# yanyan-li/Structure-SLAM-PointLine

Measured on AMD Instinct MI355X. Metric: front-end frames/sec (ORB+LSD extract+match) 640x480 @1000kp/200ln, higher is better.
Workload: dtype u8; 1 GPU; BASELINE configs[2]: 640x480 ORB(1000kp,8 levels)+LSD/LBD(<=200 lines) extract + Hamming match vs previous frame, inputs resident in HBM; batch_per_gpu=12288, global_batch=12288, unique_frames=64, streams=point branch and line branch on two HIP streams, parallelism=single GPU

## Files before the change

### include/sslam_testing.h

```cpp
#ifndef SSLAM_TESTING_H
#define SSLAM_TESTING_H
#include "sslam_frontend.h"
#ifdef __cplusplus
extern "C" {
#endif

int sslam_testing_use_rccl_standin(int on);

int sslam_selftest_exact_div(sslam_ctx* ctx, int n, long long pairs, long long* mismatches_out);
int sslam_debug_nfa_tables(int n, double* out);
int sslam_selftest_tail_test(sslam_ctx* ctx, long long samples, long long* disagree_out, long long* ambiguous_out);
int sslam_selftest_region_div(sslam_ctx* ctx, long long samples, long long mismatches_out[2]);

int sslam_selftest_sincos(sslam_ctx* ctx, long long* mismatches_out);
int sslam_selftest_lsd_bin(sslam_ctx* ctx, int max_s, long long* mismatches_out);
int sslam_selftest_lbd_round(sslam_ctx* ctx, long long mismatches_out[2]);

int sslam_selftest_valu_rate(sslam_ctx* ctx, int kind, double* ginst_per_s_out);
int sslam_selftest_fetch_probe(sslam_ctx* ctx, size_t bytes, int mode, long long* bytes_requested_out);
int sslam_lines_debug_cluster(sslam_lines* ln, int frame, long long* out8);


#ifdef __cplusplus
}
#endif
#endif
```

### structure-slam-pointline_amd/csrc/lbd.h

```cpp
#pragma once

template <class KeyPtr>
__device__ __forceinline__ void keyline_sort(KeyPtr keys, int P2, int tid) {
    for (int k = 2; k <= P2; k <<= 1)
        for (int j = k >> 1; j > 0; j >>= 1) {
            for (int i = tid; i < P2; i += 256) {
                int ixj = i ^ j;
                if (ixj > i) {
                    unsigned long long a = keys[i], c = keys[ixj];
                    bool up = (i & k) == 0;
                    if ((a > c) == up) { keys[i] = c; keys[ixj] = a; }
                }
            }
            __syncthreads();
        }
}

constexpr int KL_LDS = 1024;
__global__ __launch_bounds__(256) void k_keylines(uint8_t* __restrict__ ws, LsdPlan P, int maxLines,
                                                  sslam_keyline* __restrict__ klOut, double* __restrict__ fnOut,
                                                  int* __restrict__ counts, int cap) {
    __shared__ unsigned long long keysL[KL_LDS];
    const int b = blockIdx.x, tid = threadIdx.x;
    uint8_t* base = ws + (size_t)b * P.frameBytes;
// ... 33 lines not shown
        const float W = (float)P.w, H = (float)P.h;
        if (e0 < 0) e0 = 0; if (e0 >= W) e0 = W - 1.0f;
        if (e2 < 0) e2 = 0; if (e2 >= W) e2 = W - 1.0f;
        if (e1 < 0) e1 = 0; if (e1 >= H) e1 = H - 1.0f;
        if (e3 < 0) e3 = 0; if (e3 >= H) e3 = H - 1.0f;
        sslam_keyline k;
        k.startPointX = e0; k.startPointY = e1; k.endPointX = e2; k.endPointY = e3;
        k.sPointInOctaveX = e0; k.sPointInOctaveY = e1; k.ePointInOctaveX = e2; k.ePointInOctaveY = e3;
        const double ddx = (double)__fsub_rn(e0, e2), ddy = (double)__fsub_rn(e1, e3);
        k.lineLength = (float)sqrt(ddx * ddx + ddy * ddy);
        const int ax = cv_roundf(e0), ay = cv_roundf(e1), bx = cv_roundf(e2), by = cv_roundf(e3);
        k.numOfPixels = max(abs(bx - ax), abs(by - ay)) + 1;
        k.angle = (float)atan2((double)__fsub_rn(e3, e1), (double)__fsub_rn(e2, e0));
        k.class_id = i; k.octave = 0;
        k.size = __fmul_rn(__fsub_rn(e2, e0), __fsub_rn(e3, e1));
        k.response = __fdiv_rn(k.lineLength, (float)max(P.w, P.h));
        k.pt_x = __fdiv_rn(__fadd_rn(e2, e0), 2.f); k.pt_y = __fdiv_rn(__fadd_rn(e3, e1), 2.f);
        klw[i] = k;
        const unsigned long long key = ((unsigned long long)(~__float_as_uint(k.response)) << 32) | (unsigned)i;
        if (inLds) keysL[i] = key; else keysG[i] = key;
    }
    __syncthreads();
    int nOut = n;
    const bool doSort = n > maxLines;
    if (doSort) {
        int P2 = 1; while (P2 < n) P2 <<= 1;
        if (inLds) {
            for (int i = n + tid; i < P2; i += 256) keysL[i] = ~0ull;
            __syncthreads();
            keyline_sort(keysL, P2, tid);
        } else {
            for (int i = n + tid; i < P2; i += 256) keysG[i] = ~0ull;
            __syncthreads();
            keyline_sort(keysG, P2, tid);
        }
        nOut = maxLines;
    }
    nOut = min(nOut, cap);
    for (int i = tid; i < nOut; i += 256) {
        const int src = doSort ? (int)(unsigned)(inLds ? keysL[i] : keysG[i]) : i;
        sslam_keyline k = klw[src];
        if (doSort) k.class_id = i;
        klOut[(size_t)b * cap + i] = k;
        ((float2*)(base + P.offLbdDir))[i] = make_float2((float)cos((double)k.angle), (float)sin((double)k.angle));
        const double sx = k.startPointX, sy = k.startPointY, ex = k.endPointX, ey = k.endPointY;
        const double l0 = __dsub_rn(sy, ey), l1 = __dsub_rn(ex, sx), l2 = __dsub_rn(__dmul_rn(sx, ey), __dmul_rn(sy, ex));
        const double nrm = sqrt(__dadd_rn(__dmul_rn(l0, l0), __dmul_rn(l1, l1)));
        double* f = fnOut + ((size_t)b * cap + i) * 3;
        f[0] = l0 / nrm; f[1] = l1 / nrm; f[2] = l2 / nrm;
    }
    if (tid == 0) { counts[b] = nOut; misc->nKl = nOut; }
}

__global__ __launch_bounds__(256) void k_blur_sobel(const uint8_t* __restrict__ src, size_t spitch, size_t sframe, int w, int h,
                                                    unsigned* __restrict__ dxyo, size_t dframeBytes,
                                                    const int* __restrict__ tapsArr) {
    constexpr int R = 3;
    const int ngroups = (w + 3) >> 2;
    const int t = blockIdx.x * 256 + threadIdx.x;
    const int strip = t / ngroups, x4 = (t - strip * ngroups) * 4, y0 = strip * STRIP;
    if (y0 >= h) return;
    const int b = blockIdx.y;
    const uint8_t* s = src + (size_t)b * sframe;
    unsigned taps[5];
#pragma unroll
    for (int k = 0; k < 5; ++k) taps[k] = (unsigned)tapsArr[k];
    const unsigned T0 = taps[0] | (taps[1] << 8) | (taps[2] << 16) | (taps[3] << 24), T1 = taps[4];
    const bool fast = x4 >= 4 && x4 + 8 <= w && ((spitch | (size_t)(uintptr_t)s) & 3) == 0;
    const bool vec = ((w & 3) == 0) && ((dframeBytes & 15) == 0);
    unsigned hb[5][6];
    int bl[3][6];
    constexpr int NR = STRIP + 2 * R;
    const bool uni = row12_uniform(s, spitch, w);
    const int x4u = uni ? x4 : 0;
    Row12 ring[ROW_AHEAD_SOBEL];
#pragma unroll
    for (int k = 0; k < ROW_AHEAD_SOBEL; ++k) ring[k] = row12_issue(s, spitch, reflect_row(y0 - R + k, h, R), x4u, w);
#pragma unroll
    for (int r = 0; r < NR; ++r) {
        if (r >= 2 * R && y0 + r - 2 * R >= h) break;
        Row12 cur = ring[r % ROW_AHEAD_SOBEL];
        if (r + ROW_AHEAD_SOBEL < NR) ring[r % ROW_AHEAD_SOBEL] = row12_issue(s, spitch, reflect_row(y0 - R + r + ROW_AHEAD_SOBEL, h, R), x4u, w);
        row12_fix(cur, x4u, w);
        if (!uni) load_row12(s, spitch, reflect_row(y0 - R + r, h, R), x4, w, fast, cur.d0, cur.d1, cur.d2);
        const unsigned d0 = cur.d0, d1 = cur.d1, d2 = cur.d2;
#pragma unroll
        for (int c = 0; c < 6; ++c) hb[r % 5][c] = hdot(d0, d1, d2, c + 1, T0, T1);
        if (r >= 4) {
            const int q = r - 4;
#pragma unroll
            for (int c = 0; c < 6; ++c) {
                unsigned acc = 0;
#pragma unroll
                for (int k = 0; k < 5; ++k) acc = __umul24(hb[(q + k) % 5][c], taps[k]) + acc;
                bl[q % 3][c] = (int)min((acc + 32768u) >> 16, 255u);
            }
            if (q >= 2) {
                const int y = y0 + q - 2;
                const int* A = bl[(q - 2) % 3];
                const int* M = bl[(q - 1) % 3];
                const int* C = bl[q % 3];
                short gx[4], gy[4];
#pragma unroll
                for (int j = 0; j < 4; ++j) {
                    gx[j] = (short)((A[j + 2] - A[j]) + 2 * (M[j + 2] - M[j]) + (C[j + 2] - C[j]));
                    gy[j] = (short)((C[j] - A[j]) + 2 * (C[j + 1] - A[j + 1]) + (C[j + 2] - A[j + 2]));
                }
                unsigned* op = (unsigned*)((uint8_t*)dxyo + (size_t)b * dframeBytes) + (size_t)y * w + x4;
                unsigned pk[4];
#pragma unroll
                for (int j = 0; j < 4; ++j) pk[j] = ((unsigned)(unsigned short)gx[j]) | ((unsigned)(unsigned short)gy[j] << 16);
                if (x4 + 3 < w && vec) *(uint4*)op = make_uint4(pk[0], pk[1], pk[2], pk[3]);
                else {
#pragma unroll
                    for (int j = 0; j < 4; ++j) if (x4 + j < w) op[j] = pk[j];
                }
            }
        }
    }
}

__constant__ float kGaussL[21];
__constant__ float kGaussL2[21];
__constant__ float kGaussG[63];
__constant__ signed char kComb[64];

typedef float f32x2 __attribute__((ext_vector_type(2)));
__device__ __forceinline__ int cvt_rpi(float x) { int r; asm("v_cvt_rpi_i32_f32 %0, %1" : "=v"(r) : "v"(x)); return r; }
__device__ __forceinline__ f32x2 pk_mul_lo(f32x2 a, f32x2 b) { f32x2 r; asm("v_pk_mul_f32 %0, %1, %2 op_sel:[0,0] op_sel_hi:[1,0]" : "=v"(r) : "v"(a), "v"(b)); return r; }
__device__ __forceinline__ f32x2 pk_mul_hi_swapped(f32x2 a, f32x2 b) { f32x2 r; asm("v_pk_mul_f32 %0, %1, %2 op_sel:[1,1] op_sel_hi:[0,1]" : "=v"(r) : "v"(a), "v"(b)); return r; }
__device__ __forceinline__ f32x2 pk_add_sub(f32x2 a, f32x2 b) { f32x2 r; asm("v_pk_add_f32 %0, %1, %2 neg_hi:[0,1]" : "=v"(r) : "v"(a), "v"(b)); return r; }
__device__ __forceinline__ f32x2 pk_sub(f32x2 a, f32x2 b) { f32x2 r; asm("v_pk_add_f32 %0, %1, %2 neg_lo:[0,1] neg_hi:[0,1]" : "=v"(r) : "v"(a), "v"(b)); return r; }
__device__ __forceinline__ float max0(float x) { float r; asm("v_max_f32 %0, 0, %1" : "=v"(r) : "v"(x)); return r; }
__device__ __forceinline__ int med3_0(int x, int hi) { int r; asm("v_med3_i32 %0, %1, 0, %2" : "=v"(r) : "v"(x), "s"(hi)); return r; }
__device__ __forceinline__ f32x2 pk_mul(f32x2 a, f32x2 b) { f32x2 r; asm("v_pk_mul_f32 %0, %1, %2" : "=v"(r) : "v"(a), "v"(b)); return r; }
__device__ __forceinline__ f32x2 pk_add(f32x2 a, f32x2 b) { f32x2 r; asm("v_pk_add_f32 %0, %1, %2" : "=v"(r) : "v"(a), "v"(b)); return r; }

#ifdef SSLAM_TESTING
__global__ __launch_bounds__(256) void k_selftest_lbd_round(unsigned long long* __restrict__ bad) {
    unsigned long long nb0 = 0, nb1 = 0;
    const unsigned base = (blockIdx.x * 256u + threadIdx.x) << 8;
    for (unsigned i = 0; i < 256u; ++i) {
        const float x = __uint_as_float(base + i);
        if (!(fabsf(x) < 24608.f)) continue;
        const int t = (int)__fadd_rn(x, x);
        const int o = (int)(short)((t + 1) >> 1), n = cvt_rpi(x);
        const int Ws[3] = {0, 639, 16383};
#pragma unroll
        for (int k = 0; k < 3; ++k) nb0 += (min(max(o, 0), Ws[k]) != min(max(n, 0), Ws[k])) ? 1 : 0;
        if (x >= 0.f) nb1 += (n != (int)roundf(x)) ? 1 : 0;
    }
    if (nb0) atomicAdd(bad, nb0);
    if (nb1) atomicAdd(bad + 1, nb1);
}
#endif
constexpr int LBD_TB = 8;
template <bool RPI>
__global__ __launch_bounds__(64) void k_lbd(const uint8_t* __restrict__ ws, LsdPlan P, const sslam_keyline* __restrict__ kls,
                                            const int* __restrict__ counts, uint8_t* __restrict__ descOut, int cap) {
    constexpr int TB = LBD_TB, TN = TB, TP = TB + 1;
    __shared__ unsigned tbuf[64 * TP];
    float (*rows)[64] = (float (*)[64])&tbuf[0];
    static_assert(8 * 64 <= 64 * TP, "rows[][] lies over the walk's block array");
    __shared__ float band[8][NUM_BANDS];
    __shared__ float des[72];
    const int li = blockIdx.x, b = blockIdx.y, lane = threadIdx.x;
    if (li >= counts[b]) return;
    const uint8_t* base = ws + (size_t)b * P.frameBytes;
    const unsigned* dxyImg = (const unsigned*)(base + P.offDxy);
    const sslam_keyline kl = kls[(size_t)b * cap + li];
    const int lengthOfLSP = (short)kl.numOfPixels;
// ... 177 lines not shown
```

### structure-slam-pointline_amd/csrc/lines.hip

```cpp
#include "common.h"
#include <cmath>
#include <cstdlib>
#include <cfloat>
#include <algorithm>

namespace sslam { int launch_nfa_stream(sslam_ctx* ctx, hipStream_t st, uint8_t* ws, const void* plan, size_t planBytes, const double* lgam, uint8_t* clArea, size_t clFrameBytes,
                                        size_t stageOff, int nframes, int waves, long long spinTicks, bool besideCore); }
namespace sslam { int launch_nfa_stage(sslam_ctx* ctx, hipStream_t st, uint8_t* ws, const void* plan, size_t planBytes, const double* lgam, int nframes); }

using namespace sslam;

namespace {

#include "lsd_plan.h"
#include "lsd_front.h"
#include "lsd_regions.h"
#include "lsd_cluster.h"
#include "lsd_nfa.h"
#include "lbd.h"

__global__ void k_zero_misc(uint8_t* ws, LsdPlan P) {
    Misc* m = (Misc*)(ws + (size_t)blockIdx.x * P.frameBytes + P.offMisc);
    if (threadIdx.x == 0) {
        m->maxS = 0; m->nDefined = 0; m->nSeg = 0; m->nCand = 0; m->nKl = 0; m->overflow = 0; m->claim = 0;
#if defined(SSLAM_LSD_DRIFT_VERIFY) || defined(SSLAM_LSD_CYCLES)
        m->cyc[5] = 0; m->cyc[6] = 0; m->cyc[7] = 0;
#endif
    }
}

__global__ __launch_bounds__(256) void k_lines_status(const uint8_t* __restrict__ ws, LsdPlan P, int nframes, int maxLines, int cap, int* __restrict__ status) {
    __shared__ int cnt[2], first[2];
    if (threadIdx.x < 2) { cnt[threadIdx.x] = 0; first[threadIdx.x] = 0x7FFFFFFF; }
    __syncthreads();
    for (int b = threadIdx.x; b < nframes; b += 256) {
        const Misc* m = (const Misc*)(ws + (size_t)b * P.frameBytes + P.offMisc);
        if (min(m->nSeg, maxLines) > cap) { atomicAdd(&cnt[0], 1); atomicMin(&first[0], b); }
        if (m->overflow) { atomicAdd(&cnt[1], 1); atomicMin(&first[1], b); }
    }
    __syncthreads();
    if (threadIdx.x == 0) { status[0] = cnt[0]; status[1] = first[0]; status[2] = cnt[1]; status[3] = first[1]; }
}

}

struct sslam_lines {
    sslam_ctx* ctx;
    int maxLines;
    int planW = 0, planH = 0;
    LsdPlan plan;
    DevBuf dWs, dTabs, dTaps, dLgam, dGtab;
    size_t clFrame = 0; int clSlots = 0;
    DevBuf dCl;
    int wsFrames = 0, lastFrames = 0;
    hipEvent_t coreEvent = nullptr;
    hipEvent_t coreWait = nullptr, coreDone = nullptr;
    int lastN = -1;
    DevBuf dImg, dKl, dDesc, dFn, dCounts;
    HostPinned hOut;
    bool constsUploaded = false;
    int blurVariant = 0;
    int nfaVariant = 1, lbdBitOrder = 1, lsdResize = 0;
    int seedOrder = 0;
    int sMin = 0;
    bool fusedGeometry = false;
    hipStream_t nfaStream = nullptr; hipEvent_t nfaFork = nullptr, nfaJoin = nullptr;
};

static std::vector<int> taps_q8(int n, double sigma) {
    std::vector<double> k(n);
    double sum = 0, s2 = -0.5 / (sigma * sigma);
    for (int i = 0; i < n; ++i) { double x = i - (n - 1) * 0.5; k[i] = std::exp(s2 * x * x); sum += k[i]; }
    std::vector<int> t(n);
    double err = 0; long isum = 0;
    for (int i = 0; i < n / 2; ++i) {
        double adj = k[i] / sum * 256.0 + err;
        int v = (int)lrint(adj);
        err = adj - v; t[i] = t[n - 1 - i] = v; isum += v;
    }
    t[n / 2] = (int)(256 - 2 * isum);
    return t;
}

static std::vector<int> taps_340(int n, double sigma) {
    std::vector<float> k(n); double sum = 0; const double s2 = -0.5 / (sigma * sigma);
    for (int i = 0; i < n; ++i) { const double x = i - (n - 1) * 0.5; k[i] = (float)std::exp(s2 * x * x); sum += k[i]; }
    sum = 1. / sum;
    std::vector<int> t(n);
    for (int i = 0; i < n; ++i) { k[i] = (float)(k[i] * sum); t[i] = (int)lrint((double)k[i] * 256.0); }
    return t;
}

static size_t align_up(size_t v, size_t a) { return (v + a - 1) / a * a; }

static int lines_build_plan(sslam_lines* L, int w, int h) {
    LsdPlan& P = L->plan;
    memset(&P, 0, sizeof(P));
    P.w = w; P.h = h;
    const double SCALE = 0.8;
    P.sw = (int)lrint(w * SCALE); P.sh = (int)lrint(h * SCALE);
    if (P.sw < 8 || P.sh < 8) { set_error("image %dx%d too small for LSD", w, h); return SSLAM_ERR_UNSUPPORTED; }
    P.spitch = (P.sw + 63) & ~63;
    P.npx = P.sw * P.sh;
    if (P.sw > 65535 || P.sh > 65535) { set_error("image %dx%d too large", w, h); return SSLAM_ERR_UNSUPPORTED; }
    P.nXB = (P.sw + 255) / 256;
    P.tileRows = std::min(64, std::max(1, TILE_PX / P.sw));
    P.nTiles = (P.sh + P.tileRows - 1) / P.tileRows;
    if (P.tileRows * P.nXB > MAX_TSEG) { set_error("image %dx%d: too many segments per counting-sort tile", w, h); return SSLAM_ERR_UNSUPPORTED; }
    const double ANG_TH = 22.5, QUANT = 2.0, SIGMA_SCALE = 0.6;
    P.prec = kPI * ANG_TH / 180; P.p = ANG_TH / 180;
    P.rho = QUANT / std::sin(P.prec);
    P.logNT = 5 * (std::log10((double)P.sw) + std::log10((double)P.sh)) / 2 + std::log10(11.0);
    P.minRegSize = (int)(size_t)(-P.logNT / std::log10(P.p));
    const double sigma = SIGMA_SCALE / SCALE;
    const unsigned hk = (unsigned)std::ceil(sigma * std::sqrt(2 * 3.0 * std::log(10.0)));
    if (hk != 3) { set_error("unexpected LSD kernel size"); return SSLAM_ERR_UNSUPPORTED; }
    std::vector<int> t7 = L->blurVariant == 1 ? taps_340(7, sigma) : taps_q8(7, sigma), t5 = L->blurVariant == 1 ? taps_340(5, 1.0) : taps_q8(5, 1.0);
    for (int t : t7) if (t < 0 || t > 255) { set_error("blur taps do not fit a byte"); return SSLAM_ERR_UNSUPPORTED; }
    for (int t : t5) if (t < 0 || t > 255) { set_error("blur taps do not fit a byte"); return SSLAM_ERR_UNSUPPORTED; }
// ... 144 lines not shown
    int nfaStreamWaves;
    long long nfaSpinTicks;
};
static LinesKnobs lines_knobs() {
    LinesKnobs K{-1, true, 0, 10, 640 / CL_SUB, 0, 16, 5000000};
    if (const char* e = getenv("SSLAM_LSD_FLAVOUR")) { K.lone = e[0] == 'l' || e[0] == 'c'; K.cluster = e[0] == 'c'; }
    if (const char* e = getenv("SSLAM_LSD_CLUSTER")) K.cluster = K.cluster && atoi(e) != 0;
    if (const char* e = getenv("SSLAM_LSD_PERSIST")) { const int g = atoi(e) & ~7; if (g >= 8) K.persist = g; }
    if (const char* e = getenv("SSLAM_CL_WGS")) K.clWgs = std::max(1, std::min(CL_MAXWG, atoi(e)));
    if (const char* e = getenv("SSLAM_CL_WINDOW")) K.clWindow = std::max(-1, atoi(e));
    if (getenv("SSLAM_CL_NO_FEEDER") && K.clWindow >= 0) K.clWindow |= 1 << 20;
    if (const char* e = getenv("SSLAM_CL_SMAP")) K.clSmap = atoi(e);
    if (const char* e = getenv("SSLAM_NFA_STREAM")) { const int n = atoi(e); K.nfaStreamWaves = std::max(0, std::min(64, n == 1 ? 16 : n)); }
    if (const char* e = getenv("SSLAM_NFA_STREAM_TICKS")) K.nfaSpinTicks = std::max(0ll, atoll(e));
    return K;
}

static bool lines_guest_form(const sslam_lines* L, int nframes, const LinesKnobs& K, int* grid_out) {
    int grid = 18 * L->ctx->num_cus;
    if (2 * grid > nframes) grid = 16 * L->ctx->num_cus;
    if (K.persist) grid = K.persist;
    if (grid_out) *grid_out = grid;
    return L->coreEvent != nullptr && nframes >= 1024 && 2 * grid <= nframes;
}
extern "C" int sslam_lines_core_guest_form(sslam_lines* L, int nframes) {
    if (!L || nframes <= 0) return 0;
    return lines_guest_form(L, nframes, lines_knobs(), nullptr) ? 1 : 0;
}

enum class CoreForm {
    ClusterStream,
    Cluster,
    Lone,
    Guest,
    PerFrame,
    SixWave,
};

constexpr int CL_MAXFRAMES = 64;

static CoreForm lines_core_form(const sslam_lines* L, const LsdPlan& P, int nframes, const LinesKnobs& K, int* grid) {
    if (K.cluster && nframes <= CL_MAXFRAMES && P.sw <= TorusGlobal::XMASK + 1 && P.sh <= TorusGlobal::YMASK + 1)
        return K.nfaStreamWaves ? CoreForm::ClusterStream : CoreForm::Cluster;
    if (K.lone >= 0 ? K.lone != 0 : nframes < 1024) return CoreForm::Lone;
    if (lines_guest_form(L, nframes, K, grid)) return CoreForm::Guest;
    return nframes <= 16 * L->ctx->num_cus ? CoreForm::PerFrame : CoreForm::SixWave;
}

extern "C" int sslam_lines_destroy(sslam_lines* L) {
    if (!L) return SSLAM_OK;
    (void)hipSetDevice(L->ctx->device);
    (void)hipStreamSynchronize(L->ctx->stream);
    if (L->nfaStream) { (void)hipStreamSynchronize(L->nfaStream); (void)hipStreamDestroy(L->nfaStream); (void)hipEventDestroy(L->nfaFork); (void)hipEventDestroy(L->nfaJoin); }
    DevBuf* bufs[] = {&L->dWs, &L->dCl, &L->dTabs, &L->dTaps, &L->dLgam, &L->dGtab, &L->dImg, &L->dKl, &L->dDesc, &L->dFn, &L->dCounts};
    for (DevBuf* b : bufs) b->release();
    L->hOut.release();
    delete L;
    return SSLAM_OK;
}

struct LinesCall {
    sslam_lines* L; const LsdPlan& P; const uint8_t* images; size_t pitch, imageStride; int nframes; hipStream_t st; uint8_t* ws;
};

struct SideJoin {
    sslam_lines* L; hipStream_t st; bool forked = false, joined = false;
    void join() { if (forked && !joined) { (void)hipEventRecord(L->nfaJoin, L->nfaStream); (void)hipStreamWaitEvent(st, L->nfaJoin, 0); joined = true; } }
    ~SideJoin() { join(); }
};

static int lines_side_stream_ready(sslam_lines* L) {
    if (!L->nfaStream) {
        SSLAM_HIP(hipStreamCreateWithFlags(&L->nfaStream, hipStreamNonBlocking));
        SSLAM_HIP(hipEventCreateWithFlags(&L->nfaFork, hipEventDisableTiming));
        SSLAM_HIP(hipEventCreateWithFlags(&L->nfaJoin, hipEventDisableTiming));
    }
    return SSLAM_OK;
}

static void lines_blur_sobel(const LinesCall& c, hipStream_t s) {
    const LsdPlan& P = c.P;
    sslam::ProfScope _ps(c.L->ctx, "k_blur_sobel", s);
    hipLaunchKernelGGL(k_blur_sobel, dim3((((P.w + 3) / 4) * ((P.h + STRIP - 1) / STRIP) + 255) / 256, c.nframes), dim3(256), 0, s, c.images, c.pitch, c.imageStride, P.w, P.h,
                       (unsigned*)(c.ws + P.offDxy), P.frameBytes, c.L->dTaps.as<int>() + 8);
}

static int lines_prologue(const LinesCall& c) {
    sslam_lines* L = c.L; const LsdPlan& P = c.P; hipStream_t st = c.st;
    const int* taps = L->dTaps.as<int>();
    const int* tabX = L->dTabs.as<int>() + P.tabX; const int* tabY = L->dTabs.as<int>() + P.tabY;
    const int mode = (P.lsdResize ? 1 : 0) | (L->seedOrder ? 2 : 0);
    const bool fused = L->fusedGeometry && GRAD_ROWS == 8 && ((uintptr_t)c.images & 3) == 0 && (c.pitch & 3) == 0 && (c.imageStride & 3) == 0 && c.pitch <= 0x7FFFFFFF;
    if (fused) {
        static decltype(&k_lsd_grad_fused<0>) const kGradFused[4] = {k_lsd_grad_fused<0>, k_lsd_grad_fused<1>, k_lsd_grad_fused<2>, k_lsd_grad_fused<3>};
        sslam::ProfScope _ps(L->ctx, "k_lsd_grad", st);
        const dim3 gg(P.nXB, (P.sh + 31) / 32, c.nframes);
        hipLaunchKernelGGL(kGradFused[mode], gg, dim3(64, 4), 0, st, c.images, c.pitch, c.imageStride, c.ws, P, L->dGtab.as<float4>(), tabX, tabY, taps, c.nframes);
    } else {
        static decltype(&k_lsd_grad<0>) const kGrad[4] = {k_lsd_grad<0>, k_lsd_grad<1>, k_lsd_grad<2>, k_lsd_grad<3>};
        const size_t bpitch = ((size_t)P.w + 63) & ~(size_t)63;
        { sslam::ProfScope _ps(L->ctx, "k_blur7", st); hipLaunchKernelGGL(k_blur7, dim3((((P.w + 3) / 4) * ((P.h + STRIP - 1) / STRIP) + 255) / 256, c.nframes), dim3(256), 0, st, c.images, c.pitch, c.imageStride,
                           c.ws + P.offBlur, bpitch, P.frameBytes, P.w, P.h, taps); }
        { sslam::ProfScope _ps(L->ctx, "k_lsd_grad", st);
          const dim3 gg(P.nXB, (P.sh + 4 * GRAD_ROWS - 1) / (4 * GRAD_ROWS), c.nframes);
          hipLaunchKernelGGL(kGrad[mode], gg, dim3(64, 4), 0, st, c.ws, P, L->dGtab.as<float4>(), bpitch, tabX, tabY); }
    }
    if (L->seedOrder) return lines_host_seed_order(L, c.ws, c.nframes, st);
    const bool runs = P.sw <= (1 << SORT_XY_BITS) && P.sh <= (1 << SORT_XY_BITS);
    const dim3 sg(sort_grid(P.nTiles, c.nframes));
    { sslam::ProfScope _ps(L->ctx, "k_lsd_hist", st); hipLaunchKernelGGL(runs ? k_lsd_hist_sort : k_lsd_hist, sg, dim3(64), 0, st, c.ws, P, c.nframes); }
    { sslam::ProfScope _ps(L->ctx, "k_lsd_scan", st); hipLaunchKernelGGL(k_lsd_scan, dim3(c.nframes), dim3(1024), 0, st, c.ws, P); }
    { sslam::ProfScope _ps(L->ctx, "k_lsd_scatter", st); hipLaunchKernelGGL(runs ? k_lsd_scatter_runs : k_lsd_scatter, sg, dim3(64), 0, st, c.ws, P, c.nframes); }
    return SSLAM_OK;
}

static int lines_core_cluster(const LinesCall& c, const LinesKnobs& K, bool streamNfa, SideJoin& side, size_t* nfaStageOff) {
    sslam_lines* L = c.L; const LsdPlan& P = c.P; const int nframes = c.nframes; hipStream_t st = c.st;
    int rc;
    const bool bigFrame = P.sw > TorusFrame::XMASK + 1 || P.sh > TorusFrame::YMASK + 1;
    const int window = K.clWindow, clShift = K.clSmap;
    int nWG = K.clWgs;
    const int clSpecWords = clShift < 0 ? 0 : (((P.sw + (1 << clShift) - 1) >> clShift) * ((P.sh + (1 << clShift) - 1) >> clShift) + 31) / 32;
    const size_t maxSubs = ((size_t)P.npx + CL_SUB - 1) / CL_SUB;
    const size_t zeroBytes = 512 + ((maxSubs * sizeof(ClSub) + 511) & ~(size_t)511) + 4 * (size_t)((clSpecWords + 127) & ~127) + (bigFrame ? 4 * (size_t)TorusGlobal::WORDS : 0);
    if (nframes > 8) nWG = std::max(2, std::min(nWG, 32 / ((nframes + 7) / 8)));
    const size_t stageOff = zeroBytes + maxSubs * CL_RES * sizeof(ClRec) + 4 * (size_t)CL_ARENA * (size_t)std::max(1, (nWG - 1) * CL_HPW);
    const size_t clFrame = align_up(stageOff + (streamNfa ? sizeof(double) * 12 * (size_t)MAX_SEG : 0), 4096);
    L->clFrame = clFrame; L->clSlots = nframes;
    const size_t clSlots = (size_t)nframes;
    if (L->dCl.cap < clFrame * clSlots) { SSLAM_HIP(hipStreamSynchronize(st)); if ((rc = L->dCl.ensure(clFrame * clSlots))) return rc; }
    for (int f = 0; f < nframes; ++f) SSLAM_HIP(hipMemsetAsync(L->dCl.as<uint8_t>() + (size_t)f * clFrame, 0, zeroBytes, st));
    const size_t clLds = sizeof(unsigned) * std::max((size_t)QCAP + 4 + (bigFrame ? 0 : TorusFrame::WORDS) + CL_SCAN + CL_RING_WORDS, (size_t)CL_HPW * (CL_LIST + ClTorus::WORDS));
    const auto kern = streamNfa ? k_lsd_regions_cl<1> : k_lsd_regions_cl<0>;
    const dim3 grd(8 * nWG * ((nframes + 7) / 8));
    SSLAM_HIP(hipFuncSetAttribute((const void*)kern, hipFuncAttributeMaxDynamicSharedMemorySize, (int)clLds));
    if (!streamNfa) {
        hipLaunchKernelGGL(kern, grd, dim3(64 * CL_WAVES), clLds, st, c.ws, P, L->dCl.as<uint8_t>(), clFrame, nframes, nWG, clSpecWords, clShift, window);
        return SSLAM_OK;
    }
    if ((rc = lines_side_stream_ready(L))) return rc;
    SSLAM_HIP(hipEventRecord(L->nfaFork, st));
    hipLaunchKernelGGL(kern, grd, dim3(64 * CL_WAVES), clLds, st, c.ws, P, L->dCl.as<uint8_t>(), clFrame, nframes, nWG, clSpecWords, clShift, window);
    SSLAM_HIP(hipStreamWaitEvent(L->nfaStream, L->nfaFork, 0));
    side.forked = true;
    lines_blur_sobel(c, L->nfaStream);
    if ((rc = sslam::launch_nfa_stream(L->ctx, L->nfaStream, c.ws, &P, sizeof(P), L->dLgam.as<double>(), L->dCl.as<uint8_t>(), clFrame, stageOff, nframes, K.nfaStreamWaves, K.nfaSpinTicks, true))) return rc;
    *nfaStageOff = stageOff;
    return SSLAM_OK;
}

static int lines_core(const LinesCall& c, const LinesKnobs& K, CoreForm form, int grid, SideJoin& side, size_t* nfaStageOff) {
    sslam_lines* L = c.L; const LsdPlan& P = c.P; const int nframes = c.nframes; hipStream_t st = c.st;
    static_assert(sizeof(unsigned) * (QCAP + 4) <= 48 * 1024, "k_lsd_regions: the region queue must fit the default dynamic LDS limit (SSLAM_LSD_QCAP)");
    const size_t lds = sizeof(unsigned) * (QCAP + 4);
    if (L->coreWait) SSLAM_HIP(hipStreamWaitEvent(st, L->coreWait, 0));
    if (L->coreEvent) SSLAM_HIP(hipEventRecord(L->coreEvent, st));
    {
        sslam::ProfScope _ps(L->ctx, "k_lsd_regions", st);
        const double* lgam = L->dLgam.as<double>();
        switch (form) {
            case CoreForm::ClusterStream:
            case CoreForm::Cluster: { const int rc = lines_core_cluster(c, K, form == CoreForm::ClusterStream, side, nfaStageOff); if (rc) return rc; break; }
            case CoreForm::Lone: hipLaunchKernelGGL((k_lsd_regions<true, 4>), dim3(nframes), dim3(64), lds, st, c.ws, P, lgam, nframes); break;
            case CoreForm::Guest: hipLaunchKernelGGL((k_lsd_regions<false, 4>), dim3(grid), dim3(64), lds, st, c.ws, P, lgam, nframes); break;
            case CoreForm::PerFrame: hipLaunchKernelGGL((k_lsd_regions<false, 4>), dim3(nframes), dim3(64), lds, st, c.ws, P, lgam, nframes); break;
            case CoreForm::SixWave: hipLaunchKernelGGL((k_lsd_regions<false, 6>), dim3(nframes), dim3(64), lds, st, c.ws, P, lgam, nframes); break;
        }
    }
    if (L->coreDone) SSLAM_HIP(hipEventRecord(L->coreDone, st));
    return SSLAM_OK;
}

static int lines_tail(const LinesCall& c, CoreForm form, size_t nfaStageOff, SideJoin& side, sslam_keyline* d_kl, uint8_t* d_ldesc, double* d_linefn, int32_t* d_counts, int cap) {
    sslam_lines* L = c.L; const LsdPlan& P = c.P; const int nframes = c.nframes; hipStream_t st = c.st;
    int rc;
    if (!side.forked && nframes >= 1024 && !L->coreEvent) {
        if ((rc = lines_side_stream_ready(L))) return rc;
        SSLAM_HIP(hipEventRecord(L->nfaFork, st));
        SSLAM_HIP(hipStreamWaitEvent(L->nfaStream, L->nfaFork, 0));
        side.forked = true;
        lines_blur_sobel(c, L->nfaStream);
    }
    if (form == CoreForm::ClusterStream) {
        side.join();
        if ((rc = sslam::launch_nfa_stream(L->ctx, st, c.ws, &P, sizeof(P), L->dLgam.as<double>(), L->dCl.as<uint8_t>(), L->clFrame, nfaStageOff, nframes, 16, 0, false))) return rc;
    } else if ((rc = sslam::launch_nfa_stage(L->ctx, st, c.ws, &P, sizeof(P), L->dLgam.as<double>(), nframes))) return rc;
    { sslam::ProfScope _ps(L->ctx, "k_keylines", st); hipLaunchKernelGGL(k_keylines, dim3(nframes), dim3(256), 0, st, c.ws, P, L->maxLines, d_kl, d_linefn, d_counts, cap); }
    if (!side.forked) lines_blur_sobel(c, st);
    side.join();
    {
        const bool rpi = P.w <= 16384 && P.h <= 16384;
        sslam::ProfScope _ps(L->ctx, "k_lbd", st);
        hipLaunchKernelGGL(rpi ? k_lbd<true> : k_lbd<false>, dim3(std::min(L->maxLines, cap), nframes), dim3(64), 0, st, c.ws, P, d_kl, d_counts, d_ldesc, cap);
    }
    return SSLAM_OK;
}

extern "C" int sslam_lines_extract_batch_dev(sslam_lines* L, const uint8_t* d_images, int w, int h, size_t pitch, size_t image_stride,
                                             int nframes, sslam_keyline* d_kl, uint8_t* d_ldesc, double* d_linefn, int32_t* d_counts,
                                             int cap, void* stream_) {
    if (!L || !d_images || !d_kl || !d_ldesc || !d_linefn || !d_counts || w <= 0 || h <= 0 || nframes <= 0 || cap <= 0 || pitch < (size_t)w) {
        set_error("sslam_lines_extract_batch_dev: invalid arguments"); return SSLAM_ERR_INVALID;
    }
    const LinesKnobs K = lines_knobs();
    std::lock_guard<std::recursive_mutex> lk(L->ctx->mu);
    SSLAM_HIP(hipSetDevice(L->ctx->device));
    hipStream_t st = stream_ ? (hipStream_t)stream_ : L->ctx->stream;
    int rc;
    if (w != L->planW || h != L->planH) { SSLAM_HIP(hipStreamSynchronize(st)); if ((rc = lines_build_plan(L, w, h))) return rc; }
    if (!L->constsUploaded) {
        float gl[21], gg[63];
        {
            double u = (BAND_W * 3 - 1) / 2, sigma = (BAND_W * 2 + 1) / 2, inv = -1 / (2 * sigma * sigma);
            for (int i = 0; i < 21; ++i) { double d = i - u; gl[i] = (float)std::exp(d * d * inv); }
            u = (NUM_BANDS * BAND_W - 1) / 2; sigma = u; inv = -1 / (2 * sigma * sigma);
            for (int i = 0; i < 63; ++i) { double d = i - u; gg[i] = (float)std::exp(d * d * inv); }
        }
        static const signed char comb[64] = {0, 1, 0, 2, 0, 3, 0, 4, 0, 5, 0, 6, 1, 2, 1, 3, 1, 4, 1, 5, 1, 6, 2, 3, 2, 4, 2, 5, 2, 6, 2, 7,
                                             2, 8, 3, 4, 3, 5, 3, 6, 3, 7, 3, 8, 4, 5, 4, 6, 4, 7, 4, 8, 5, 6, 5, 7, 5, 8, 6, 7, 6, 8, 7, 8};
        float gl2[21];
        for (int i = 0; i < 21; ++i) { volatile float c = gl[i]; gl2[i] = c * c; }
        SSLAM_HIP(hipMemcpyToSymbol(HIP_SYMBOL(kGaussL), gl, sizeof(gl)));
        SSLAM_HIP(hipMemcpyToSymbol(HIP_SYMBOL(kGaussL2), gl2, sizeof(gl2)));
        SSLAM_HIP(hipMemcpyToSymbol(HIP_SYMBOL(kGaussG), gg, sizeof(gg)));
        SSLAM_HIP(hipMemcpyToSymbol(HIP_SYMBOL(kComb), comb, sizeof(comb)));
        L->constsUploaded = true;
    }
    const LsdPlan& P = L->plan;
    if (nframes > L->wsFrames) {
        SSLAM_HIP(hipStreamSynchronize(st));
        if ((rc = L->dWs.ensure(P.frameBytes * (size_t)nframes))) return rc;
        L->wsFrames = nframes;
    }
    const LinesCall c{L, P, d_images, pitch, image_stride, nframes, st, L->dWs.as<uint8_t>()};
    { sslam::ProfScope _ps(L->ctx, "k_zero_misc", st); hipLaunchKernelGGL(k_zero_misc, dim3(nframes), dim3(64), 0, st, c.ws, P); }
    SideJoin side{L, st};
    if ((rc = lines_prologue(c))) return rc;
    int grid = 0;
    const CoreForm form = lines_core_form(L, P, nframes, K, &grid);
    size_t nfaStageOff = 0;
    if ((rc = lines_core(c, K, form, grid, side, &nfaStageOff))) return rc;
// ... 189 lines not shown
        double s0, c0, s1, c1;
        sincos((double)x, &s0, &c0); sslam::sincos_0_2pi((double)x, s1, c1);
        if (__float_as_uint((float)s0) != __float_as_uint((float)s1) || __float_as_uint((float)c0) != __float_as_uint((float)c1)) ++nb;
    }
    if (nb) atomicAdd(bad, nb);
}
}
extern "C" int sslam_selftest_sincos(sslam_ctx* ctx, long long* mismatches_out) {
    if (!ctx || !mismatches_out) return SSLAM_ERR_INVALID;
    SSLAM_HIP(hipSetDevice(ctx->device));
    ScopedDev dMem;
    SSLAM_HIP(hipMalloc(&dMem.p, sizeof(unsigned long long)));
    unsigned long long* d = (unsigned long long*)dMem.p;
    SSLAM_HIP(hipMemset(d, 0, sizeof(unsigned long long)));
    const unsigned nthreads = (0x40D00000u >> 6) + 1;
    hipLaunchKernelGGL(k_selftest_sincos, dim3((nthreads + 255) / 256), dim3(256), 0, ctx->stream, d);
    unsigned long long h = 0;
    SSLAM_HIP(hipMemcpyAsync(&h, d, sizeof(h), hipMemcpyDeviceToHost, ctx->stream));
    SSLAM_HIP(hipStreamSynchronize(ctx->stream));
    *mismatches_out = (long long)h;
    return SSLAM_OK;
}

extern "C" int sslam_selftest_lsd_bin(sslam_ctx* ctx, int max_s, long long* mismatches_out) {
    if (!ctx || max_s < 0 || max_s >= (1 << 24) || !mismatches_out) return SSLAM_ERR_INVALID;
    SSLAM_HIP(hipSetDevice(ctx->device));
    ScopedDev dMem;
    SSLAM_HIP(hipMalloc(&dMem.p, sizeof(unsigned long long)));
    unsigned long long* d = (unsigned long long*)dMem.p;
    SSLAM_HIP(hipMemset(d, 0, sizeof(unsigned long long)));
    hipLaunchKernelGGL(k_selftest_lsd_bin, dim3(2048), dim3(256), 0, ctx->stream, max_s, d);
    unsigned long long h = 0;
    SSLAM_HIP(hipMemcpyAsync(&h, d, sizeof(h), hipMemcpyDeviceToHost, ctx->stream));
    SSLAM_HIP(hipStreamSynchronize(ctx->stream));
    *mismatches_out = (long long)h;
    return SSLAM_OK;
}

extern "C" int sslam_selftest_lbd_round(sslam_ctx* ctx, long long* mismatches_out) {
    if (!ctx || !mismatches_out) return SSLAM_ERR_INVALID;
    SSLAM_HIP(hipSetDevice(ctx->device));
    ScopedDev dMem;
    SSLAM_HIP(hipMalloc(&dMem.p, 2 * sizeof(unsigned long long)));
    unsigned long long* d = (unsigned long long*)dMem.p;
    SSLAM_HIP(hipMemset(d, 0, 2 * sizeof(unsigned long long)));
    hipLaunchKernelGGL(k_selftest_lbd_round, dim3(65536), dim3(256), 0, ctx->stream, d);
    unsigned long long h[2] = {0, 0};
    SSLAM_HIP(hipMemcpyAsync(h, d, sizeof(h), hipMemcpyDeviceToHost, ctx->stream));
    SSLAM_HIP(hipStreamSynchronize(ctx->stream));
    mismatches_out[0] = (long long)h[0]; mismatches_out[1] = (long long)h[1];
    return SSLAM_OK;
}

namespace {
template <int KIND>
__global__ __launch_bounds__(256) void k_probe_valu(int iters, unsigned* __restrict__ sink) {
    unsigned a[16]; double d[16];
#pragma unroll
    for (int i = 0; i < 16; ++i) { a[i] = threadIdx.x + i; d[i] = (double)(threadIdx.x + i); }
    const unsigned b = blockIdx.x | 1u; const float fb = 1.0000001f; const double db = 1e-9;
    for (int it = 0; it < iters; ++it) {
#pragma unroll
        for (int i = 0; i < 16; ++i) {
            if (KIND == 0) asm volatile("v_add_u32 %0, %0, %1" : "+v"(a[i]) : "v"(b));
            else if (KIND == 1) asm volatile("v_fma_f32 %0, %0, %1, %1" : "+v"(a[i]) : "v"(fb));
            else if (KIND == 2) asm volatile("v_add_f64 %0, %0, %1" : "+v"(d[i]) : "v"(db));
            else asm volatile("v_bcnt_u32_b32 %0, %1, %0" : "+v"(a[i]) : "v"(b));
        }
    }
    unsigned acc = 0;
#pragma unroll
    for (int i = 0; i < 16; ++i) acc += a[i] + (unsigned)d[i];
    if (acc == 0x12345u) *sink = acc;
}
}
extern "C" int sslam_selftest_valu_rate(sslam_ctx* ctx, int kind, double* ginst_per_s_out) {
    if (!ctx || kind < 0 || kind > 3 || !ginst_per_s_out) return SSLAM_ERR_INVALID;
    SSLAM_HIP(hipSetDevice(ctx->device));
    ScopedDev sinkMem;
    SSLAM_HIP(hipMalloc(&sinkMem.p, 4));
    const int blocks = ctx->num_cus * 8, iters = 20000;
    hipEvent_t e0, e1;
    SSLAM_HIP(hipEventCreate(&e0)); SSLAM_HIP(hipEventCreate(&e1));
    for (int rep = 0; rep < 2; ++rep) {
        (void)hipEventRecord(e0, ctx->stream);
        if (kind == 0) hipLaunchKernelGGL(k_probe_valu<0>, dim3(blocks), dim3(256), 0, ctx->stream, iters, (unsigned*)sinkMem.p);
        else if (kind == 1) hipLaunchKernelGGL(k_probe_valu<1>, dim3(blocks), dim3(256), 0, ctx->stream, iters, (unsigned*)sinkMem.p);
        else if (kind == 2) hipLaunchKernelGGL(k_probe_valu<2>, dim3(blocks), dim3(256), 0, ctx->stream, iters, (unsigned*)sinkMem.p);
        else hipLaunchKernelGGL(k_probe_valu<3>, dim3(blocks), dim3(256), 0, ctx->stream, iters, (unsigned*)sinkMem.p);
        (void)hipEventRecord(e1, ctx->stream);
        if (hipStreamSynchronize(ctx->stream) != hipSuccess) { (void)hipEventDestroy(e0); (void)hipEventDestroy(e1); set_error("sslam_selftest_valu_rate: kernel failed"); return SSLAM_ERR_HIP; }
    }
    float ms = 0; (void)hipEventElapsedTime(&ms, e0, e1);
    (void)hipEventDestroy(e0); (void)hipEventDestroy(e1);
    *ginst_per_s_out = (double)blocks * 4.0 * iters * 16.0 / (ms * 1e-3) / 1e9;
    return SSLAM_OK;
}

extern "C" int sslam_selftest_fetch_probe(sslam_ctx* ctx, size_t bytes, int mode, long long* bytes_requested_out) {
    if (!ctx || bytes < (1u << 20) || (mode != 0 && mode != 1) || !bytes_requested_out) return SSLAM_ERR_INVALID;
    SSLAM_HIP(hipSetDevice(ctx->device));
    ScopedDev bufMem, sinkMem;
    SSLAM_HIP(hipMalloc(&bufMem.p, bytes));
    SSLAM_HIP(hipMalloc(&sinkMem.p, sizeof(float)));
    float4* buf = (float4*)bufMem.p; float* sink = (float*)sinkMem.p;
    SSLAM_HIP(hipMemsetAsync(buf, 0, bytes, ctx->stream));
// ... 61 lines not shown
```

### structure-slam-pointline_amd/csrc/lsd_front.h

```cpp
#pragma once

constexpr int STRIP = 32;

__device__ __forceinline__ void load_row12(const uint8_t* __restrict__ s, size_t spitch, int yy, int x4, int w, bool fast, unsigned& d0, unsigned& d1, unsigned& d2) {
    const uint8_t* row = s + (size_t)yy * spitch;
    if (fast) {
        const unsigned* q = (const unsigned*)(row + x4 - 4);
        d0 = q[0]; d1 = q[1]; d2 = q[2];
    } else {
        unsigned px[12];
#pragma unroll
        for (int i = 0; i < 12; ++i) {
            int xx = reflect101(min(x4 - 4 + i, w + 2), w);
            xx = min(max(xx, 0), w - 1);
            px[i] = row[xx];
        }
        d0 = px[0] | (px[1] << 8) | (px[2] << 16) | (px[3] << 24);
        d1 = px[4] | (px[5] << 8) | (px[6] << 16) | (px[7] << 24);
        d2 = px[8] | (px[9] << 8) | (px[10] << 16) | (px[11] << 24);
    }
}
struct Row12 { unsigned d0, d1, d2; };
constexpr int ROW_AHEAD_BLUR7 = 1, ROW_AHEAD_SOBEL = 2;
__device__ __forceinline__ bool row12_uniform(const uint8_t* s, size_t spitch, int w) { return (w & 3) == 0 && w >= 12 && ((spitch | (size_t)(uintptr_t)s) & 3) == 0; }
__device__ __forceinline__ Row12 row12_issue(const uint8_t* __restrict__ s, size_t spitch, int yy, int x4, int w) {
    const unsigned* q = (const unsigned*)(s + (size_t)yy * spitch + x4);
    Row12 r; r.d1 = q[0]; r.d0 = q[x4 < 4 ? 0 : -1]; r.d2 = q[x4 + 8 > w ? 0 : 1];
    return r;
}
__device__ __forceinline__ void row12_fix(Row12& r, int x4, int w) {
    const unsigned l = __builtin_amdgcn_perm(r.d2, r.d1, 0x01020304u);
    const unsigned rr = __builtin_amdgcn_perm(r.d1, r.d0, 0x03040506u);
    r.d0 = x4 < 4 ? l : r.d0; r.d2 = x4 + 8 > w ? rr : r.d2;
}
__device__ __forceinline__ unsigned hdot(unsigned d0, unsigned d1, unsigned d2, int s, unsigned T0, unsigned T1) {
    const unsigned lo = s < 4 ? __builtin_amdgcn_alignbyte(d1, d0, (unsigned)s) : __builtin_amdgcn_alignbyte(d2, d1, (unsigned)(s - 4));
    const unsigned hi = s < 4 ? __builtin_amdgcn_alignbyte(d2, d1, (unsigned)s) : (d2 >> (8 * (s - 4)));
    return __builtin_amdgcn_udot4(lo, T0, __builtin_amdgcn_udot4(hi, T1, 0u, false), false);
}
__device__ __forceinline__ int reflect_row(int y, int h, int R) {
    const int yy = reflect101(min(y, h + R - 1), h);
    return min(max(yy, 0), h - 1);
}

__global__ __launch_bounds__(256) void k_blur7(const uint8_t* __restrict__ src, size_t spitch, size_t sframe,
                                               uint8_t* __restrict__ dst, size_t dpitch, size_t dframe, int w, int h,
                                               const int* __restrict__ tapsArr) {
    constexpr int R = 3;
    const int ngroups = (w + 3) >> 2;
    const int t = blockIdx.x * 256 + threadIdx.x;
    const int strip = t / ngroups, x4 = (t - strip * ngroups) * 4, y0 = strip * STRIP;
    if (y0 >= h) return;
    const int b = blockIdx.y;
    const uint8_t* s = src + (size_t)b * sframe;
    uint8_t* d = dst + (size_t)b * dframe;
    unsigned taps[7];
#pragma unroll
    for (int k = 0; k < 7; ++k) taps[k] = (unsigned)tapsArr[k];
    const unsigned T0 = taps[0] | (taps[1] << 8) | (taps[2] << 16) | (taps[3] << 24), T1 = taps[4] | (taps[5] << 8) | (taps[6] << 16);
    const bool fast = x4 >= 4 && x4 + 8 <= w && ((spitch | (size_t)(uintptr_t)s) & 3) == 0;
    unsigned win[7][4];
    constexpr int NR = STRIP + 2 * R;
    const bool uni = row12_uniform(s, spitch, w);
    const int x4u = uni ? x4 : 0;
    Row12 ring[ROW_AHEAD_BLUR7];
#pragma unroll
    for (int k = 0; k < ROW_AHEAD_BLUR7; ++k) ring[k] = row12_issue(s, spitch, reflect_row(y0 - R + k, h, R), x4u, w);
#pragma unroll
    for (int r = 0; r < NR; ++r) {
        if (r >= 2 * R && y0 + r - 2 * R >= h) break;
        Row12 cur = ring[r % ROW_AHEAD_BLUR7];
        if (r + ROW_AHEAD_BLUR7 < NR) ring[r % ROW_AHEAD_BLUR7] = row12_issue(s, spitch, reflect_row(y0 - R + r + ROW_AHEAD_BLUR7, h, R), x4u, w);
        row12_fix(cur, x4u, w);
        if (!uni) load_row12(s, spitch, reflect_row(y0 - R + r, h, R), x4, w, fast, cur.d0, cur.d1, cur.d2);
        const unsigned d0 = cur.d0, d1 = cur.d1, d2 = cur.d2;
#pragma unroll
// ... 625 lines not shown
```

Measured before the change: 81790 frames/s.

## Roll blur-sobel row loop with register shift window and dedicated low-priority stream

Rewrites k_blur_sobel so the row loop is no longer fully unrolled. It keeps a 4-deep horizontal-blur window and a 2-row blur window in shifted registers, prefetches only one row ahead, and templates on uniform alignment with a higher occupancy launch bound. This is meant to cut register pressure and code size so more waves fit per CU. Blur-sobel also moves off the NFA side stream onto its own low-priority stream, so it can overlap the NFA stage even when a core event is present, and an optional path can fork it under the core stage. The rolled loop adds per-row register copy overhead, and the 8-waves launch bound may force spills.

Measured after the change: 82900 frames/s, median of 6. 1.4% higher.

```diff
diff --git a/include/sslam_testing.h b/include/sslam_testing.h
--- a/include/sslam_testing.h
+++ b/include/sslam_testing.h
@@ -16,6 +16,9 @@
 int sslam_selftest_lsd_bin(sslam_ctx* ctx, int max_s, long long* mismatches_out);
 int sslam_selftest_lbd_round(sslam_ctx* ctx, long long mismatches_out[2]);
 
+int sslam_testing_lbd_gradient(sslam_ctx* ctx, const uint8_t* img, int w, int h, size_t pitch, size_t image_stride, int nframes, int offset, int variant,
+                               uint32_t* dxy_out);
+
 int sslam_selftest_valu_rate(sslam_ctx* ctx, int kind, double* ginst_per_s_out);
 int sslam_selftest_fetch_probe(sslam_ctx* ctx, size_t bytes, int mode, long long* bytes_requested_out);
 int sslam_lines_debug_cluster(sslam_lines* ln, int frame, long long* out8);
diff --git a/structure-slam-pointline_amd/csrc/lbd.h b/structure-slam-pointline_amd/csrc/lbd.h
--- a/structure-slam-pointline_amd/csrc/lbd.h
+++ b/structure-slam-pointline_amd/csrc/lbd.h
@@ -109,9 +109,10 @@
     if (tid == 0) { counts[b] = nOut; misc->nKl = nOut; }
 }
 
-__global__ __launch_bounds__(256) void k_blur_sobel(const uint8_t* __restrict__ src, size_t spitch, size_t sframe, int w, int h,
-                                                    unsigned* __restrict__ dxyo, size_t dframeBytes,
-                                                    const int* __restrict__ tapsArr) {
+template <bool UNI>
+__global__ __launch_bounds__(256, UNI ? 8 : 4) void k_blur_sobel(const uint8_t* __restrict__ src, size_t spitch, size_t sframe, int w, int h,
+                                                       unsigned* __restrict__ dxyo, size_t dframeBytes,
+                                                       const int* __restrict__ tapsArr) {
     constexpr int R = 3;
     const int ngroups = (w + 3) >> 2;
     const int t = blockIdx.x * 256 + threadIdx.x;
@@ -125,45 +126,41 @@
     const unsigned T0 = taps[0] | (taps[1] << 8) | (taps[2] << 16) | (taps[3] << 24), T1 = taps[4];
     const bool fast = x4 >= 4 && x4 + 8 <= w && ((spitch | (size_t)(uintptr_t)s) & 3) == 0;
     const bool vec = ((w & 3) == 0) && ((dframeBytes & 15) == 0);
-    unsigned hb[5][6];
-    int bl[3][6];
-    constexpr int NR = STRIP + 2 * R;
-    const bool uni = row12_uniform(s, spitch, w);
+    unsigned* op = (unsigned*)((uint8_t*)dxyo + (size_t)b * dframeBytes) + (size_t)y0 * w + x4;
+    unsigned hb0[6], hb1[6], hb2[6], hb3[6];
+    int blA[6], blM[6];
+    const int nr = min(STRIP + 2 * R, h - y0 + 2 * R);
+    const bool uni = UNI || row12_uniform(s, spitch, w);
     const int x4u = uni ? x4 : 0;
-    Row12 ring[ROW_AHEAD_SOBEL];
-#pragma unroll
-    for (int k = 0; k < ROW_AHEAD_SOBEL; ++k) ring[k] = row12_issue(s, spitch, reflect_row(y0 - R + k, h, R), x4u, w);
-#pragma unroll
-    for (int r = 0; r < NR; ++r) {
-        if (r >= 2 * R && y0 + r - 2 * R >= h) break;
-        Row12 cur = ring[r % ROW_AHEAD_SOBEL];
-        if (r + ROW_AHEAD_SOBEL < NR) ring[r % ROW_AHEAD_SOBEL] = row12_issue(s, spitch, reflect_row(y0 - R + r + ROW_AHEAD_SOBEL, h, R), x4u, w);
+    auto srow = [h](int y) { int yy = y < 0 ? -y : y; yy = yy >= h ? 2 * h - 2 - yy : yy; yy = yy < 0 ? -yy : yy; return min(yy, h - 1); };
+    Row12 next = row12_issue(s, spitch, srow(y0 - R), x4u, w);
+#pragma unroll 1
+    for (int r = 0; r < nr; ++r) {
+        Row12 cur = next;
+        if (r + 1 < nr) next = row12_issue(s, spitch, srow(y0 - R + r + 1), x4u, w);
         row12_fix(cur, x4u, w);
-        if (!uni) load_row12(s, spitch, reflect_row(y0 - R + r, h, R), x4, w, fast, cur.d0, cur.d1, cur.d2);
-        const unsigned d0 = cur.d0, d1 = cur.d1, d2 = cur.d2;
-#pragma unroll
-        for (int c = 0; c < 6; ++c) hb[r % 5][c] = hdot(d0, d1, d2, c + 1, T0, T1);
+        if (!uni) load_row12(s, spitch, srow(y0 - R + r), x4, w, fast, cur.d0, cur.d1, cur.d2);
+        unsigned hn[6];
+#pragma unroll
+        for (int c = 0; c < 6; ++c) hn[c] = hdot(cur.d0, cur.d1, cur.d2, c + 1, T0, T1);
         if (r >= 4) {
-            const int q = r - 4;
+            int bn[6];
 #pragma unroll
             for (int c = 0; c < 6; ++c) {
-                unsigned acc = 0;
-#pragma unroll
-                for (int k = 0; k < 5; ++k) acc = __umul24(hb[(q + k) % 5][c], taps[k]) + acc;
-                bl[q % 3][c] = (int)min((acc + 32768u) >> 16, 255u);
-            }
-            if (q >= 2) {
-                const int y = y0 + q - 2;
-                const int* A = bl[(q - 2) % 3];
-                const int* M = bl[(q - 1) % 3];
-                const int* C = bl[q % 3];
+                unsigned acc = __umul24(hb0[c], taps[0]);
+                acc = __umul24(hb1[c], taps[1]) + acc;
+                acc = __umul24(hb2[c], taps[2]) + acc;
+                acc = __umul24(hb3[c], taps[3]) + acc;
+                acc = __umul24(hn[c], taps[4]) + acc;
+                bn[c] = (int)min((acc + 32768u) >> 16, 255u);
+            }
+            if (r >= 6) {
                 short gx[4], gy[4];
 #pragma unroll
                 for (int j = 0; j < 4; ++j) {
-                    gx[j] = (short)((A[j + 2] - A[j]) + 2 * (M[j + 2] - M[j]) + (C[j + 2] - C[j]));
-                    gy[j] = (short)((C[j] - A[j]) + 2 * (C[j + 1] - A[j + 1]) + (C[j + 2] - A[j + 2]));
+                    gx[j] = (short)((blA[j + 2] - blA[j]) + 2 * (blM[j + 2] - blM[j]) + (bn[j + 2] - bn[j]));
+                    gy[j] = (short)((bn[j] - blA[j]) + 2 * (bn[j + 1] - blA[j + 1]) + (bn[j + 2] - blA[j + 2]));
                 }
-                unsigned* op = (unsigned*)((uint8_t*)dxyo + (size_t)b * dframeBytes) + (size_t)y * w + x4;
                 unsigned pk[4];
 #pragma unroll
                 for (int j = 0; j < 4; ++j) pk[j] = ((unsigned)(unsigned short)gx[j]) | ((unsigned)(unsigned short)gy[j] << 16);
@@ -172,8 +169,13 @@
 #pragma unroll
                     for (int j = 0; j < 4; ++j) if (x4 + j < w) op[j] = pk[j];
                 }
-            }
-        }
+                op += w;
+            }
+#pragma unroll
+            for (int c = 0; c < 6; ++c) { blA[c] = blM[c]; blM[c] = bn[c]; }
+        }
+#pragma unroll
+        for (int c = 0; c < 6; ++c) { hb0[c] = hb1[c]; hb1[c] = hb2[c]; hb2[c] = hb3[c]; hb3[c] = hn[c]; }
     }
 }
 
diff --git a/structure-slam-pointline_amd/csrc/lines.hip b/structure-slam-pointline_amd/csrc/lines.hip
--- a/structure-slam-pointline_amd/csrc/lines.hip
+++ b/structure-slam-pointline_amd/csrc/lines.hip
@@ -65,6 +65,7 @@
     int sMin = 0;
     bool fusedGeometry = false;
     hipStream_t nfaStream = nullptr; hipEvent_t nfaFork = nullptr, nfaJoin = nullptr;
+    hipStream_t blurStream = nullptr; hipEvent_t blurFork = nullptr, blurJoin = nullptr;
 };
 
 static std::vector<int> taps_q8(int n, double sigma) {
@@ -315,6 +316,7 @@
     (void)hipSetDevice(L->ctx->device);
     (void)hipStreamSynchronize(L->ctx->stream);
     if (L->nfaStream) { (void)hipStreamSynchronize(L->nfaStream); (void)hipStreamDestroy(L->nfaStream); (void)hipEventDestroy(L->nfaFork); (void)hipEventDestroy(L->nfaJoin); }
+    if (L->blurStream) { (void)hipStreamSynchronize(L->blurStream); (void)hipStreamDestroy(L->blurStream); (void)hipEventDestroy(L->blurFork); (void)hipEventDestroy(L->blurJoin); }
     DevBuf* bufs[] = {&L->dWs, &L->dCl, &L->dTabs, &L->dTaps, &L->dLgam, &L->dGtab, &L->dImg, &L->dKl, &L->dDesc, &L->dFn, &L->dCounts};
     for (DevBuf* b : bufs) b->release();
     L->hOut.release();
@@ -327,8 +329,11 @@
 };
 
 struct SideJoin {
-    sslam_lines* L; hipStream_t st; bool forked = false, joined = false;
-    void join() { if (forked && !joined) { (void)hipEventRecord(L->nfaJoin, L->nfaStream); (void)hipStreamWaitEvent(st, L->nfaJoin, 0); joined = true; } }
+    sslam_lines* L; hipStream_t st; bool forked = false, joined = false, blurForked = false, blurJoined = false;
+    void join() {
+        if (forked && !joined) { (void)hipEventRecord(L->nfaJoin, L->nfaStream); (void)hipStreamWaitEvent(st, L->nfaJoin, 0); joined = true; }
+        if (blurForked && !blurJoined) { (void)hipEventRecord(L->blurJoin, L->blurStream); (void)hipStreamWaitEvent(st, L->blurJoin, 0); blurJoined = true; }
+    }
     ~SideJoin() { join(); }
 };
 
@@ -341,11 +346,31 @@
     return SSLAM_OK;
 }
 
+static void launch_blur_sobel(const uint8_t* images, size_t pitch, size_t imageStride, int w, int h, int nframes, unsigned* dxy, size_t dframeBytes, const int* taps5,
+                              hipStream_t s) {
+    const bool uni = (w & 3) == 0 && w >= 12 && (((uintptr_t)images | pitch | imageStride) & 3) == 0;
+    hipLaunchKernelGGL(uni ? k_blur_sobel<true> : k_blur_sobel<false>, dim3((((w + 3) / 4) * ((h + STRIP - 1) / STRIP) + 255) / 256, nframes), dim3(256), 0, s,
+                       images, pitch, imageStride, w, h, dxy, dframeBytes, taps5);
+}
 static void lines_blur_sobel(const LinesCall& c, hipStream_t s) {
     const LsdPlan& P = c.P;
     sslam::ProfScope _ps(c.L->ctx, "k_blur_sobel", s);
-    hipLaunchKernelGGL(k_blur_sobel, dim3((((P.w + 3) / 4) * ((P.h + STRIP - 1) / STRIP) + 255) / 256, c.nframes), dim3(256), 0, s, c.images, c.pitch, c.imageStride, P.w, P.h,
-                       (unsigned*)(c.ws + P.offDxy), P.frameBytes, c.L->dTaps.as<int>() + 8);
+    launch_blur_sobel(c.images, c.pitch, c.imageStride, P.w, P.h, c.nframes, (unsigned*)(c.ws + P.offDxy), P.frameBytes, c.L->dTaps.as<int>() + 8, s);
+}
+static int lines_fork_blur_sobel(const LinesCall& c, SideJoin& side) {
+    sslam_lines* L = c.L;
+    if (!L->blurStream) {
+        int least = 0, greatest = 0;
+        SSLAM_HIP(hipDeviceGetStreamPriorityRange(&least, &greatest));
+        SSLAM_HIP(hipStreamCreateWithPriority(&L->blurStream, hipStreamNonBlocking, least));
+        SSLAM_HIP(hipEventCreateWithFlags(&L->blurFork, hipEventDisableTiming));
+        SSLAM_HIP(hipEventCreateWithFlags(&L->blurJoin, hipEventDisableTiming));
+    }
+    SSLAM_HIP(hipEventRecord(L->blurFork, c.st));
+    SSLAM_HIP(hipStreamWaitEvent(L->blurStream, L->blurFork, 0));
+    side.blurForked = true;
+    lines_blur_sobel(c, L->blurStream);
+    return SSLAM_OK;
 }
 
 static int lines_prologue(const LinesCall& c) {
@@ -418,6 +443,9 @@
     const size_t lds = sizeof(unsigned) * (QCAP + 4);
     if (L->coreWait) SSLAM_HIP(hipStreamWaitEvent(st, L->coreWait, 0));
     if (L->coreEvent) SSLAM_HIP(hipEventRecord(L->coreEvent, st));
+#ifdef SSLAM_SOBEL_UNDER_CORE
+    if (form == CoreForm::Guest) { const int rc = lines_fork_blur_sobel(c, side); if (rc) return rc; }
+#endif
     {
         sslam::ProfScope _ps(L->ctx, "k_lsd_regions", st);
         const double* lgam = L->dLgam.as<double>();
@@ -437,19 +465,14 @@
 static int lines_tail(const LinesCall& c, CoreForm form, size_t nfaStageOff, SideJoin& side, sslam_keyline* d_kl, uint8_t* d_ldesc, double* d_linefn, int32_t* d_counts, int cap) {
     sslam_lines* L = c.L; const LsdPlan& P = c.P; const int nframes = c.nframes; hipStream_t st = c.st;
     int rc;
-    if (!side.forked && nframes >= 1024 && !L->coreEvent) {
-        if ((rc = lines_side_stream_ready(L))) return rc;
-        SSLAM_HIP(hipEventRecord(L->nfaFork, st));
-        SSLAM_HIP(hipStreamWaitEvent(L->nfaStream, L->nfaFork, 0));
-        side.forked = true;
-        lines_blur_sobel(c, L->nfaStream);
-    }
+    if (!side.forked && !side.blurForked && nframes >= 1024)
+        if ((rc = lines_fork_blur_sobel(c, side))) return rc;
     if (form == CoreForm::ClusterStream) {
         side.join();
         if ((rc = sslam::launch_nfa_stream(L->ctx, st, c.ws, &P, sizeof(P), L->dLgam.as<double>(), L->dCl.as<uint8_t>(), L->clFrame, nfaStageOff, nframes, 16, 0, false))) return rc;
     } else if ((rc = sslam::launch_nfa_stage(L->ctx, st, c.ws, &P, sizeof(P), L->dLgam.as<double>(), nframes))) return rc;
     { sslam::ProfScope _ps(L->ctx, "k_keylines", st); hipLaunchKernelGGL(k_keylines, dim3(nframes), dim3(256), 0, st, c.ws, P, L->maxLines, d_kl, d_linefn, d_counts, cap); }
-    if (!side.forked) lines_blur_sobel(c, st);
+    if (!side.forked && !side.blurForked) lines_blur_sobel(c, st);
     side.join();
     {
         const bool rpi = P.w <= 16384 && P.h <= 16384;
@@ -745,6 +768,29 @@
     return SSLAM_OK;
 }
 
+extern "C" int sslam_testing_lbd_gradient(sslam_ctx* ctx, const uint8_t* img, int w, int h, size_t pitch, size_t image_stride, int nframes, int offset, int variant,
+                                          uint32_t* dxy_out) {
+    if (!ctx || !img || !dxy_out || w <= 0 || h <= 0 || nframes <= 0 || offset < 0 || pitch < (size_t)w || image_stride < pitch * (size_t)h || (variant != 0 && variant != 1))
+        return SSLAM_ERR_INVALID;
+    SSLAM_HIP(hipSetDevice(ctx->device));
+    const std::vector<int> t5 = variant == 1 ? taps_340(5, 1.0) : taps_q8(5, 1.0);
+    const size_t srcBytes = (size_t)offset + image_stride * (size_t)nframes, planeBytes = sizeof(unsigned) * (size_t)w * h;
+    ScopedDev dSrc, dOut, dTaps;
+    SSLAM_HIP(hipMalloc(&dSrc.p, srcBytes));
+    SSLAM_HIP(hipMalloc(&dOut.p, planeBytes * nframes));
+    SSLAM_HIP(hipMalloc(&dTaps.p, sizeof(int) * 5));
+    SSLAM_HIP(hipMemset(dSrc.p, 0, srcBytes));
+    uint8_t* src = (uint8_t*)dSrc.p + offset;
+    for (int f = 0; f < nframes; ++f)
+        SSLAM_HIP(hipMemcpy2D(src + (size_t)f * image_stride, pitch, img, pitch, (size_t)w, (size_t)h, hipMemcpyHostToDevice));
+    SSLAM_HIP(hipMemcpy(dTaps.p, t5.data(), sizeof(int) * 5, hipMemcpyHostToDevice));
+    launch_blur_sobel(src, pitch, image_stride, w, h, nframes, (unsigned*)dOut.p, planeBytes, (const int*)dTaps.p, ctx->stream);
+    SSLAM_HIP(hipGetLastError());
+    SSLAM_HIP(hipMemcpyAsync(dxy_out, dOut.p, planeBytes * nframes, hipMemcpyDeviceToHost, ctx->stream));
+    SSLAM_HIP(hipStreamSynchronize(ctx->stream));
+    return SSLAM_OK;
+}
+
 namespace {
 template <int KIND>
 __global__ __launch_bounds__(256) void k_probe_valu(int iters, unsigned* __restrict__ sink) {
diff --git a/structure-slam-pointline_amd/csrc/lsd_front.h b/structure-slam-pointline_amd/csrc/lsd_front.h
--- a/structure-slam-pointline_amd/csrc/lsd_front.h
+++ b/structure-slam-pointline_amd/csrc/lsd_front.h
@@ -21,7 +21,7 @@
     }
 }
 struct Row12 { unsigned d0, d1, d2; };
-constexpr int ROW_AHEAD_BLUR7 = 1, ROW_AHEAD_SOBEL = 2;
+constexpr int ROW_AHEAD_BLUR7 = 1;
 __device__ __forceinline__ bool row12_uniform(const uint8_t* s, size_t spitch, int w) { return (w & 3) == 0 && w >= 12 && ((spitch | (size_t)(uintptr_t)s) & 3) == 0; }
 __device__ __forceinline__ Row12 row12_issue(const uint8_t* __restrict__ s, size_t spitch, int yy, int x4, int w) {
     const unsigned* q = (const unsigned*)(s + (size_t)yy * spitch + x4);
```
